# danspeech/danspeech

Hardware: AMD Instinct MI355X
Metric: audio-seconds/sec (RTFx) recognize() on 10 s clips, batch=32 (higher is better)
Workload: dtype f32 (two-term fp16 split operands, 3 MFMA products, fp32 accumulate)

## Files before the change

### danspeech_amd/csrc/api.hip

```cpp
#include "common.h"
#include "model.h"

#include <algorithm>
#include <cmath>
#include <cstring>
#include <cstdlib>
#include <mutex>
#include <fcntl.h>
#include <sys/file.h>
#include <unistd.h>

using namespace dsmi;

static thread_local std::string g_create_error;

#define HIP_OK(m, expr)                                                                   \
    do {                                                                                  \
        hipError_t e_ = (expr);                                                           \
        if (e_ != hipSuccess) {                                                           \
            (m)->err = std::string(#expr) + ": " + hipGetErrorString(e_);                 \
            return DSMI_ERR_HIP;                                                          \
        }                                                                                 \
    } while (0)

// ... 601 lines not shown
        return RingEnv{k && std::string(k) == "ring4", t ? std::atoi(t) : 4, c ? std::atoi(c) : 0};
    }();
    return env;
}

static RnnPlanInput rnn_plan_input(const dsmi_model* m, int B, bool split16) {
    RnnPlanInput in;
    in.geom = m->geom; in.geom16 = m->geom16; in.have16 = m->have16; in.split16 = split16;
    in.B = B; in.n_cus = m->n_cus; in.inflight = m->inflight; in.ring_windows = m->ring_windows; in.lane = m->lane;
    in.rnn_mode = m->rnn_mode; in.persist_gen = m->persist_gen; in.rnn_kernel = m->rnn_kernel; in.ring8 = m->ring8; in.ring4 = m->ring4;
    in.ring4_small_shapes = ring_env().small_shapes; in.ring4_most = ring_env().most; in.ring_slot_cap = ring_env().slot_cap;
    return in;
}

static bool run_rnn_plan(dsmi_model* m, const RnnPlan& plan, int l, int B, int To, int dst, double sumlen, hipStream_t s) {
    const double H = m->desc.rnn_hidden_size, GH = (double)m->geom.G * m->desc.rnn_hidden_size, Dd = m->geom.D;
    if (plan.launches[0].kernel == RNN_STEPS) {
        RnnStepLaunch st = rnn_step_launch(m, l, B, To, dst);
        for (int step = 0; step < To; ++step) {
            st.step = step;
            int act = 0;
            for (int i = 0; i < B; ++i) act += step < m->host_out_lens[i] ? 1 : 0;
            st.ev = timer_arm(m, KK_STEP, (step & 7) == 3, 2.0 * Dd * GH * H * act, 4.0 * Dd * (GH * H + (double)B * (GH + 2.0 * H)));
            launch_rnn_step(st, s);
        }
        m->last_plan_x16 = false; m->last_plan_n = 1; m->last_plan[0] = plan.launches[0];
        return true;
    }
    RnnPersist16Launch p16;
    RnnPersistLaunch p8;
    if (plan.x16) p16 = persist16_launch(m, l, B, To, dst);
    else p8 = persist_launch(m, l, B, To, dst);
    const size_t cnt_words = (size_t)m->geom.D * ceil_div(B, 16) * To * kPersist16CntWords;
    if (plan.x16) (void)hipMemsetAsync(m->pcnt, 0, sizeof(unsigned) * (cnt_words + 2 * ceil_div(B, 16) + 2), s);
    else (void)hipMemsetAsync(m->pcnt, 0, sizeof(unsigned) * (size_t)m->geom.D * ceil_div(B, 32) * To, s);
    static const bool ring_xcd = [] { const char* e = exp_env("DSMI_DEBUG_RING_XCD"); return !(e && e[0] == '0'); }();
    PersistGate* gate = persist_gate(m->device);
    std::unique_lock<std::mutex> turn(gate->mu, std::defer_lock);
    bool ok = true;
    for (int i = 0; i < plan.launches.size() && ok; ++i) {
        const RnnLaunch& L = plan.launches[i];
        const EvPair ev = timer_arm(m, KK_PERSIST, true, L.part * 2.0 * Dd * GH * H * sumlen, L.part * 4.0 * Dd * (GH * H + (double)To * B * (GH + 2.0 * H)));
        if (!L.join) {
            turn.lock();
            if (L.gate == GATE_RING) ring_gate_wait(gate, s, L.slot0, L.nslots, L.cus, m->n_cus);
            else gate_wait(gate, s, L.slot0, L.nslots);
        }
        p16.ev = ev;
        switch (L.kernel) {
            case RNN_PERSIST8: p8.ev = ev; p8.d0 = L.at; p8.ny = L.n; ok = launch_rnn_persist(p8, s); break;
            case RNN_PERSIST16: p16.pgroups = L.n; p16.waves = 8; ok = launch_rnn_persist16(p16, s); break;
            case RNN_PERSIST16_HALF: p16.pgroups = L.n; p16.waves = 4; ok = launch_rnn_persist16(p16, s); break;
            case RNN_DUO: p16.pair0 = L.at; p16.npairs = L.n; ok = launch_rnn_persist_duo(p16, s); break;
            default:
                p16.tile0 = L.at; p16.ntw = L.n; p16.nwin = L.nwin;
                p16.tickets = ring_xcd ? m->pcnt + cnt_words + L.ticket : nullptr;
                ok = L.kernel == RNN_RING8 ? launch_rnn_persist_ring(p16, s) : launch_rnn_persist_ring4(p16, s);
        }
        if (!ok || i + 1 == plan.launches.size() || !plan.launches[i + 1].join) {
            if (L.gate == GATE_RING) ring_gate_record(gate, s, L.slot0, L.nslots, L.cus);
            else gate_record(gate, s, L.slot0, L.nslots);
            turn.unlock();
        }
    }
    if (ok) {
        m->last_plan_x16 = plan.x16; m->last_plan_n = plan.launches.size();
        for (int i = 0; i < std::min(m->last_plan_n, (int)dsmi_model::kLastPlanKept); ++i) m->last_plan[i] = plan.launches[i];
    }
    return ok;
}

static void run_rnn_layer(dsmi_model* m, int l, GemmLaunch gl, int B, int To, int dst, hipStream_t s) {
    double sumlen = 0;
    for (int i = 0; i < B; ++i) sumlen += m->host_out_lens[i];
    const double GH = (double)m->geom.G * m->desc.rnn_hidden_size, Dd = m->geom.D;
    RnnPlanInput in = rnn_plan_input(m, B, m->gemm_mode == 1 && gl.w_sp);
    RnnPlan plan = plan_rnn_layer(in);
    if (plan.x16) {
        gl.w_sp = m->rnn[l].wih16_sp; gl.bias = m->rnn[l].bih16; gl.N = m->geom16.Np; gl.ldc = m->geom16.Np;
    }
    gl.ev = timer_arm(m, gl.mode == GEMM_A_CONV ? KK_GEMM0 : KK_GEMM, true, 2.0 * Dd * GH * gl.K * sumlen,
                      4.0 * ((double)gl.M * gl.K * (gl.a2 ? 2 : 1) + (double)gl.N * gl.K + (double)gl.M * gl.N));
    unsigned* sem = (dense_tokens() > 0 && m->inflight >= 2) ? dense_sem(m->device) : nullptr;
    if (sem) hipLaunchKernelGGL(dense_enter_kernel, dim3(1), dim3(64), 0, s, sem, (unsigned)dense_tokens());
    launch_gemm(gl, s);
    if (sem) hipLaunchKernelGGL(dense_leave_kernel, dim3(1), dim3(64), 0, s, sem);
    if (run_rnn_plan(m, plan, l, B, To, dst, sumlen, s)) return;
    if (plan.x16) {
        gl.w_sp = m->rnn[l].wih_sp; gl.bias = m->rnn[l].bih; gl.N = m->geom.Np; gl.ldc = m->geom.Np; gl.ev = EvPair{};
        launch_gemm(gl, s);
        in.have16 = false;
        plan = plan_rnn_layer(in);
        if (run_rnn_plan(m, plan, l, B, To, dst, sumlen, s)) return;
    }
    in.rnn_mode = 0;
    (void)run_rnn_plan(m, plan_rnn_layer(in), l, B, To, dst, sumlen, s);
}

static GemmLaunch xproj_gemm(dsmi_model* m, int l, int B, int To) {
    GemmLaunch gl{};
    const RnnW& r = m->rnn[l];
    gl.w = r.wih; gl.bias = r.bih; gl.c = m->xp;
    gl.w_sp = m->gemm_mode == 1 ? r.wih_sp : nullptr;
    gl.a_sp = m->a_sp;
    gl.M = To * B; gl.N = m->geom.Np; gl.K = r.K; gl.ldw = r.ldw; gl.ldc = m->geom.Np;
    gl.B = B; gl.T = To;
    return gl;
}

static int stage_lens(dsmi_model* m, int B, hipStream_t s) {
    if (B > m->stage_cap) {
        HIP_OK(m, hipDeviceSynchronize());
        if (m->lens_stage) (void)hipHostFree(m->lens_stage);
        m->lens_stage = nullptr;
        const int cap = std::max(B, 64);
        HIP_OK(m, hipHostMalloc((void**)&m->lens_stage, sizeof(int32_t) * (size_t)cap * dsmi_model::kStage, hipHostMallocDefault));
        m->stage_cap = cap;
        for (int i = 0; i < dsmi_model::kStage; ++i) {
            if (!m->stage_ev[i]) HIP_OK(m, hipEventCreateWithFlags(&m->stage_ev[i], hipEventDisableTiming));
            m->stage_used[i] = false;
        }
    }
    const int slot = m->stage_next++ % dsmi_model::kStage;
    if (m->stage_used[slot]) HIP_OK(m, hipEventSynchronize(m->stage_ev[slot]));
    int32_t* h = m->lens_stage + (size_t)slot * m->stage_cap;
    std::memcpy(h, m->host_out_lens.data(), sizeof(int32_t) * B);
    HIP_OK(m, hipMemcpyAsync(m->lens_dev, h, sizeof(int32_t) * B, hipMemcpyHostToDevice, s));
    HIP_OK(m, hipEventRecord(m->stage_ev[slot], s));
    m->stage_used[slot] = true;
    return DSMI_OK;
}

static int forward_enqueue(dsmi_model* m, const float* feat, int B, int T, float* probs, hipStream_t s);

static int persist_give_up(dsmi_model* m, hipStream_t s) {
    m->rnn_mode = 0;
    HIP_OK(m, hipMemsetAsync(m->perr, 0, sizeof(unsigned), s));
    return DSMI_OK;
}

static int collect_oldest(dsmi_model* m, bool recompute) {
    dsmi_model::FwdSlot& f = m->fwd[m->fwd_head];
    HIP_OK(m, hipEventSynchronize(f.done));
    m->fwd_head = (m->fwd_head + 1) % dsmi_model::kFwdRing;
    m->fwd_count -= 1;
    if (*f.err_host == 0) return DSMI_OK;
    *f.err_host = 0;
    hipStream_t s = (hipStream_t)f.stream;
    int rc;
    if ((rc = persist_give_up(m, s))) return rc;
    if (!recompute)
        return fail(m, DSMI_ERR_TIMEOUT, "the persistent recurrent kernel timed out in an earlier forward whose status was never "
                                         "collected with dsmi_forward_status: those results were invalid; this handle now runs "
                                         "one launch per step");
    m->host_out_lens.resize(f.B);
    for (int i = 0; i < f.B; ++i) m->host_out_lens[i] = seq_len(m, f.lens[i]);
    if ((rc = forward_enqueue(m, f.feat, f.B, f.T, f.probs, s))) return rc;
    HIP_OK(m, hipStreamSynchronize(s));
    m->recomputed += 1;
    m->err = "a hand-off wait of the persistent recurrent kernel timed out; the batch was recomputed with one launch per step";
    return DSMI_RECOMPUTED;
}

extern "C" int dsmi_forward(dsmi_model* m, const float* feat, const int32_t* lens, int B, int T, float* probs,
                            int32_t* out_lens, void* stream) {
    if (!m) return DSMI_ERR_INVALID;
    int rc = check_batch(m, lens, B, T);
// ... 371 lines not shown
```

### danspeech_amd/csrc/common.h

```cpp
#pragma once
#include <hip/hip_runtime.h>
#include <hip/hip_ext.h>
#include <cstdint>
#include <cstdio>
#include <cstdlib>
#include <string>
#include <vector>
#include <map>

#include "../../include/dsmi.h"
#include "rnn_plan.h"

namespace dsmi {

using f32x4 = __attribute__((ext_vector_type(4))) float;
using f32x16 = __attribute__((ext_vector_type(16))) float;

constexpr int kWave = 64;

struct EvPair { hipEvent_t start = nullptr, stop = nullptr; };
#define DSMI_LAUNCH(kern, grid, block, lds, stream, ev, ...)                                          \
    do {                                                                                              \
        if ((ev).start) hipExtLaunchKernelGGL(kern, grid, block, lds, stream, (ev).start, (ev).stop, 0, __VA_ARGS__); \
        else hipLaunchKernelGGL(kern, grid, block, lds, stream, __VA_ARGS__);                          \
    } while (0)

inline const char* exp_env(const char* name) {
#ifdef DSMI_EXPERIMENTS
    return std::getenv(name);
#else
    (void)name;
    return nullptr;
#endif
}

struct ConvSpec { int ci, co, kf, kt, sf, st, pf, pt; };
static const ConvSpec kConvSpecs[3] = {
    {1, 32, 41, 11, 2, 2, 20, 5},
    {32, 32, 21, 11, 2, 1, 10, 5},
    {32, 96, 21, 11, 2, 1, 10, 5},
};


struct ConvLaunch {
    const float* x; float* y; const float* wp; const float* bias; const float* bn_a; const float* bn_b;
    const int32_t* out_lens_dev;
    int B, ci, co, fi, fo, ti, to, xs, ys, layer;
    uint16_t* y_sp = nullptr;
    EvPair ev;
};
void launch_conv(const ConvLaunch& p, hipStream_t s);

struct ConvSplitLaunch {
    const uint16_t* x_sp;
    const uint16_t* wp_sp;
    const float* bias; const float* bn_a; const float* bn_b; const int32_t* out_lens_dev;
    float* y;
    uint16_t* y_sp;
    int B, co, fi, fo, ti, to, ys;
    EvPair ev;
};
void launch_conv_split(const ConvSplitLaunch& p, hipStream_t s);
std::vector<uint16_t> pack_conv_w_split(const float* w, int co_total);
std::vector<float> pack_conv_weights(const float* w, int layer);

std::vector<uint16_t> pack_conv1_w_split(const float* w);
void launch_conv1_split(const ConvLaunch& p, const uint16_t* wp_sp, hipStream_t s);

enum GemmAMode {
    GEMM_A_ROWMAJOR = 0,
    GEMM_A_SUM_BN = 1,
    GEMM_A_CONV = 2
};
struct GemmLaunch {
    int mode;
    const float* a; const float* a2; const float* alpha; const float* beta;
    const float* w; const float* bias; float* c;
    const uint16_t* w_sp = nullptr;
    uint16_t* a_sp = nullptr;
    int M, N, K;
    int lda, ldw, ldc;
    int B, T, ys;
    EvPair ev;
};
void launch_gemm(const GemmLaunch& p, hipStream_t s);
std::vector<uint16_t> pack_gemm_w_split(const float* w, int N, int K, int ldw);

int rnn_src_row(const RnnGeom& g, int packed_col, int* dir_out);
std::vector<float> pack_whh(const RnnGeom& g, const float* w_hh);
struct RnnStepLaunch {
    RnnGeom g;
    const float* whh_packed[2];
    const float* bhh[2];
    const float* xp;
    float* out[2];
    float* cstate[2];
    const int32_t* lens_dev;
    float* hpack;
    int B, T, step;
    const float* hcarry = nullptr;
    int pbase = 0;
    EvPair ev;
    unsigned long long* dbg = nullptr;
};
void launch_rnn_step(const RnnStepLaunch& p, hipStream_t s);

constexpr unsigned kPersistSpinLimit = 1u << 22;

struct RnnPersistLaunch {
    RnnGeom g;
    const uint16_t* whh_sp[2];
    const float* bhh[2]; const float* xp; float* out[2];
    const int32_t* lens_dev; uint16_t* hpack_sp;
    unsigned* counters;
    unsigned* err;
    int B, T;
    int d0 = 0, ny = 1;
    unsigned spin_limit = kPersistSpinLimit;
    int drop_wg = -1, drop_step = -1;
    EvPair ev;
    unsigned long long* dbg = nullptr;
    const float* h0 = nullptr;
    float* cst = nullptr;
};
std::vector<uint16_t> pack_whh_split(const RnnGeom& g, const float* w_hh);
bool launch_rnn_persist(const RnnPersistLaunch& p, hipStream_t s);

struct RnnPersist16Launch {
    RnnGeom g;
    const uint16_t* whh16[2];
    const float* bhh[2]; const float* xp; float* out[2];
    const int32_t* lens_dev; uint16_t* hpack16;
    unsigned* counters;
    unsigned* err;
    int B, T, pgroups;
    int waves = 8;
    int pair0 = 0, npairs = 0;
    int tile0 = 0, ntw = 0, nwin = 1;
    unsigned* tickets = nullptr;
    unsigned spin_limit = kPersistSpinLimit;
    int drop_wg = -1, drop_step = -1;
    EvPair ev;
    unsigned long long* dbg = nullptr;
};
constexpr int kPersist16Shards = 4;
constexpr int kPersist16CntWords = kPersist16Shards * 64;
std::vector<uint16_t> pack_whh16(const RnnGeom& g16, const float* w_hh);
size_t rnn_persist16_state_halfs(const RnnGeom& g16, int B);
bool launch_rnn_persist16(const RnnPersist16Launch& p, hipStream_t s);

bool launch_rnn_persist_duo(const RnnPersist16Launch& p, hipStream_t s);

bool launch_rnn_persist_ring(const RnnPersist16Launch& p, hipStream_t s);
bool launch_rnn_persist_ring4(const RnnPersist16Launch& p, hipStream_t s);

void launch_lookahead(const float* x, const float* w, float* y, int T, int B, int H, int context, hipStream_t s);
struct HeadLaunch {
    const float* x1; const float* x2; const float* bn_a; const float* bn_b;
    const float* w_packed; int H, C, T, B; float* probs;
    EvPair ev;
};
std::vector<float> pack_fc(const float* w, int C, int H);
void launch_head(const HeadLaunch& p, hipStream_t s);
void launch_greedy(const float* probs, const int32_t* sizes_dev, int B, int T, int C, int blank,
                   int32_t* raw, int32_t* ids, int32_t* offsets, int32_t* n_out, hipStream_t s);
void launch_add2(const float* a, const float* b, float* y, size_t rows, int H, int Hs, hipStream_t s);
void launch_pad_rows(const float* x, float* y, size_t rows, int I, int Is, hipStream_t s);
// ... 3 lines not shown
```

### danspeech_amd/csrc/conv1_split.hip

```cpp
#include "common.h"

namespace dsmi {

namespace {

using f16x8 = __attribute__((ext_vector_type(8))) _Float16;
using f16x4 = __attribute__((ext_vector_type(4))) _Float16;
using f16x2 = __attribute__((ext_vector_type(2))) _Float16;
using u32x4 = __attribute__((ext_vector_type(4))) unsigned int;
constexpr float kLoScale = 2048.f, kLoInv = 1.f / 2048.f;

constexpr int KF = 41, KT = 11, SF = 2, ST = 2, PF = 20, PT = 5, CO = 32;
constexpr int C1NF = 8;
constexpr int C1NT = C1NF * 64;
constexpr int C1TT = 64;
constexpr int ROWS = SF * (C1NF - 1) + KF;
constexpr int WIN = ST * (C1TT - 1) + KT + 5;
constexpr int PITCH = 144;
constexpr int COPY = ROWS * PITCH;
constexpr size_t C1_LDS = (size_t)2 * 2 * COPY * 2;

struct Conv1Args {
    const float* x; const uint16_t* wp; const float* bias; const float* bn_a; const float* bn_b; const int32_t* out_lens;
    float* y; uint16_t* y_sp;
    int B, fi, fo, ti, to, xs, ys;
};

template <bool SPLIT_OUT>
__global__ __launch_bounds__(C1NT, 4) void conv1_f16x3_kernel(Conv1Args p) {
    extern __shared__ __attribute__((aligned(16))) unsigned char c1sm[];
    _Float16* Xs = reinterpret_cast<_Float16*>(c1sm);
    const int tid = threadIdx.x, lane = tid & 63;
    const int wv = __builtin_amdgcn_readfirstlane(tid >> 6);
    const int li = lane & 31, hk = lane >> 5;
    const int t0 = blockIdx.x * C1TT, f0 = blockIdx.y * C1NF, b = blockIdx.z;
    const int f = f0 + wv;
    const int olen = p.out_lens[b];

    if (t0 >= olen) {
        if (SPLIT_OUT) {
            for (int idx = tid; idx < C1NF * 2 * C1TT * 4; idx += C1NT) {
                const int part = idx & 3, tl = (idx >> 2) % C1TT, pl = (idx / (4 * C1TT)) % 2, ff = idx / (4 * C1TT * 2);
                if (f0 + ff < p.fo && t0 + tl < p.to)
                    *reinterpret_cast<u32x4*>(reinterpret_cast<_Float16*>(p.y_sp) + ((((size_t)b * p.fo + f0 + ff) * 2 + pl) * p.to + t0 + tl) * 32 + part * 8) = u32x4{0, 0, 0, 0};
            }
        } else {
            for (int idx = tid; idx < CO * C1NF * C1TT; idx += C1NT) {
                const int tl = idx % C1TT, ff = (idx / C1TT) % C1NF, co = idx / (C1TT * C1NF);
                if (f0 + ff < p.fo && t0 + tl < p.to) p.y[(((size_t)b * CO + co) * p.fo + f0 + ff) * p.ys + t0 + tl] = 0.f;
            }
        }
        return;
    }

    const int fin0 = SF * f0 - PF, tin0 = ST * t0 - PT;
    for (int idx = tid; idx < ROWS * (PITCH / 2); idx += C1NT) {
        const int row = idx / (PITCH / 2), q = 2 * (idx - row * (PITCH / 2));
        const int fin = fin0 + row;
        float v[2] = {0.f, 0.f};
        if (fin >= 0 && fin < p.fi) {
            const float* src = p.x + ((size_t)b * p.fi + fin) * p.xs;
#pragma unroll
            for (int e = 0; e < 2; ++e) {
                const int tin = tin0 + q + e;
                if (tin >= 0 && tin < p.ti && q + e < WIN) v[e] = src[tin];
            }
        }
        f16x2 h, l;
#pragma unroll
        for (int e = 0; e < 2; ++e) {
            const _Float16 hi = (_Float16)v[e];
            h[e] = hi; l[e] = (_Float16)((v[e] - (float)hi) * kLoScale);
        }
        _Float16* r0 = Xs + row * PITCH + q;
        *reinterpret_cast<f16x2*>(r0) = h;
        *reinterpret_cast<f16x2*>(r0 + 2 * COPY) = l;
        if (q >= 2) {
            *reinterpret_cast<f16x2*>(r0 + COPY - 2) = h;
            *reinterpret_cast<f16x2*>(r0 + 3 * COPY - 2) = l;
        }
    }
    __syncthreads();
    if (f >= p.fo) return;

    f32x16 acc[2], acl[2];
#pragma unroll
    for (int tt = 0; tt < 2; ++tt)
#pragma unroll
        for (int r = 0; r < 16; ++r) { acc[tt][r] = 0.f; acl[tt][r] = 0.f; }

    const _Float16* xb = Xs + (SF * wv) * PITCH + 4 * li + 8 * hk;
    const u32x4* wq = reinterpret_cast<const u32x4*>(p.wp) + lane;
    u32x4 wn[2] = {wq[0], wq[64]};
#pragma unroll 1
    for (int kf = 0; kf < KF; ++kf) {
        const f16x8 wh = __builtin_bit_cast(f16x8, wn[0]), wl = __builtin_bit_cast(f16x8, wn[1]);
        if (kf + 1 < KF) { wn[0] = wq[(size_t)(kf + 1) * 128]; wn[1] = wq[(size_t)(kf + 1) * 128 + 64]; }
        const _Float16* xr = xb + kf * PITCH;
        f16x8 xh[2], xl[2];
#pragma unroll
        for (int tt = 0; tt < 2; ++tt) {
            const f16x4 a0 = *reinterpret_cast<const f16x4*>(xr + tt * COPY), a1 = *reinterpret_cast<const f16x4*>(xr + tt * COPY + 4);
            const f16x4 b0 = *reinterpret_cast<const f16x4*>(xr + (2 + tt) * COPY), b1 = *reinterpret_cast<const f16x4*>(xr + (2 + tt) * COPY + 4);
            xh[tt] = f16x8{a0[0], a0[1], a0[2], a0[3], a1[0], a1[1], a1[2], a1[3]};
            xl[tt] = f16x8{b0[0], b0[1], b0[2], b0[3], b1[0], b1[1], b1[2], b1[3]};
        }
#pragma unroll
        for (int tt = 0; tt < 2; ++tt) acl[tt] = __builtin_amdgcn_mfma_f32_32x32x16_f16(wl, xh[tt], acl[tt], 0, 0, 0);
#pragma unroll
        for (int tt = 0; tt < 2; ++tt) acc[tt] = __builtin_amdgcn_mfma_f32_32x32x16_f16(wh, xh[tt], acc[tt], 0, 0, 0);
#pragma unroll
        for (int tt = 0; tt < 2; ++tt) acl[tt] = __builtin_amdgcn_mfma_f32_32x32x16_f16(wh, xl[tt], acl[tt], 0, 0, 0);
    }

#pragma unroll
    for (int tt = 0; tt < 2; ++tt) {
        const int t = t0 + 2 * li + tt;
        if (t >= p.to) continue;
        if (SPLIT_OUT) {
#pragma unroll
            for (int g = 0; g < 4; ++g) {
                f16x4 h, l;
#pragma unroll
                for (int q = 0; q < 4; ++q) {
                    const int co = q + 8 * g + 4 * hk;
                    float v = (acc[tt][4 * g + q] + acl[tt][4 * g + q] * kLoInv + p.bias[co]) * p.bn_a[co] + p.bn_b[co];
                    v = fminf(fmaxf(v, 0.f), 20.f);
                    v = t < olen ? v : 0.f;
                    const _Float16 a = (_Float16)v;
                    h[q] = a; l[q] = (_Float16)(v - (float)a);
                }
                _Float16* base = reinterpret_cast<_Float16*>(p.y_sp) + ((((size_t)b * p.fo + f) * 2) * (size_t)p.to + t) * 32 + 8 * g + 4 * hk;
                *reinterpret_cast<f16x4*>(base) = h;
                *reinterpret_cast<f16x4*>(base + (size_t)p.to * 32) = l;
            }
        } else {
#pragma unroll
            for (int r = 0; r < 16; ++r) {
                const int co = (r & 3) + 8 * (r >> 2) + 4 * hk;
                float v = (acc[tt][r] + acl[tt][r] * kLoInv + p.bias[co]) * p.bn_a[co] + p.bn_b[co];
                v = fminf(fmaxf(v, 0.f), 20.f);
                p.y[(((size_t)b * CO + co) * p.fo + f) * p.ys + t] = t < olen ? v : 0.f;
            }
        }
    }
}

inline uint16_t c1_bits(_Float16 h) {
    uint16_t u;
    __builtin_memcpy(&u, &h, 2);
    return u;
}

}

std::vector<uint16_t> pack_conv1_w_split(const float* w) {
    std::vector<uint16_t> out((size_t)KF * 2 * 64 * 8, 0);
    for (int kf = 0; kf < KF; ++kf)
        for (int lane = 0; lane < 64; ++lane)
            for (int e = 0; e < 8; ++e) {
                const int co = lane & 31, kt = 8 * (lane >> 5) + e;
                if (kt >= KT) continue;
                const float x = w[((size_t)co * KF + kf) * KT + kt];
                const _Float16 h1 = (_Float16)x;
                const _Float16 h2 = (_Float16)((x - (float)h1) * kLoScale);
                const size_t base = (((size_t)kf * 2) * 64 + lane) * 8 + e;
                out[base] = c1_bits(h1); out[base + 512] = c1_bits(h2);
            }
    return out;
}

void launch_conv1_split(const ConvLaunch& c, const uint16_t* wp_sp, hipStream_t s) {
    Conv1Args a{c.x, wp_sp, c.bias, c.bn_a, c.bn_b, c.out_lens_dev, c.y, c.y_sp, c.B, c.fi, c.fo, c.ti, c.to, c.xs, c.ys};
    const dim3 grid(ceil_div(c.to, C1TT), ceil_div(c.fo, C1NF), c.B);
    if (c.y_sp) {
        (void)hipFuncSetAttribute(reinterpret_cast<const void*>(conv1_f16x3_kernel<true>), hipFuncAttributeMaxDynamicSharedMemorySize, (int)C1_LDS);
        DSMI_LAUNCH(conv1_f16x3_kernel<true>, grid, dim3(C1NT), C1_LDS, s, c.ev, a);
    } else {
        (void)hipFuncSetAttribute(reinterpret_cast<const void*>(conv1_f16x3_kernel<false>), hipFuncAttributeMaxDynamicSharedMemorySize, (int)C1_LDS);
        DSMI_LAUNCH(conv1_f16x3_kernel<false>, grid, dim3(C1NT), C1_LDS, s, c.ev, a);
// ... 5 lines not shown
```

### danspeech_amd/csrc/conv_split.hip

```cpp
#include "common.h"
#include <type_traits>

namespace dsmi {

namespace {

using f16x8 = __attribute__((ext_vector_type(8))) _Float16;
using f16x4 = __attribute__((ext_vector_type(4))) _Float16;
constexpr float kConvWScale = 64.f;
using u32x4 = __attribute__((ext_vector_type(4))) unsigned int;

constexpr int BNF = 4;
constexpr int BTT = 64;
constexpr int KT = 11, KF = 21, SF = 2, PF = 10, PT = 5, CI = 32;
constexpr int WIN = BTT + KT - 1;
constexpr int NPL = 2;
constexpr int PITCH = 32;
constexpr int ROWPLANE = WIN * PITCH;
constexpr int RCHUNK = NPL * WIN * 4;
constexpr int CPR = (RCHUNK + 255) / 256;
constexpr int NSLOT = 2 * BNF;

struct ConvSplitArgs {
    const uint16_t* x_sp; const uint16_t* wp_sp; const float* bias; const float* bn_a; const float* bn_b;
    const int32_t* out_lens; float* y; uint16_t* y_sp;
    int B, fi, fo, ti, to, ys;
    int nco;
};

__device__ __forceinline__ void store_split4(uint16_t* y_sp, size_t bf_index, int t_stride, int t, int c0, const float (&v)[4]) {
    f16x4 h, l;
#pragma unroll
    for (int c = 0; c < 4; ++c) {
        const _Float16 hi = (_Float16)v[c];
        h[c] = hi; l[c] = (_Float16)(v[c] - (float)hi);
    }
    _Float16* base = reinterpret_cast<_Float16*>(y_sp) + ((bf_index * NPL) * (size_t)t_stride + t) * 32 + c0;
    *reinterpret_cast<f16x4*>(base) = h;
    *reinterpret_cast<f16x4*>(base + (size_t)t_stride * 32) = l;
}

template <bool SPLIT_OUT, bool XPIPE = true>
__global__ __launch_bounds__(256, 2) void conv_f16x3_kernel(ConvSplitArgs p) {
    extern __shared__ __attribute__((aligned(16))) unsigned char csm[];
    _Float16* Xs = reinterpret_cast<_Float16*>(csm);
    const int tid = threadIdx.x, lane = tid & 63;
    const int wv = __builtin_amdgcn_readfirstlane(tid >> 6);
    const int t0 = blockIdx.x * BTT, f0 = blockIdx.y * BNF;
    const int b = blockIdx.z / p.nco, ct = blockIdx.z - b * p.nco;
    const int f = f0 + wv;
    const int olen = p.out_lens[b];
    const int CO = 32 * p.nco;

    if (t0 >= olen) {
        if (SPLIT_OUT) {
            for (int idx = tid; idx < BNF * NPL * BTT * 4; idx += 256) {
                const int part = idx & 3, tl = (idx >> 2) % BTT, pl = (idx / (4 * BTT)) % NPL, ff = idx / (4 * BTT * NPL);
                if (f0 + ff < p.fo && t0 + tl < p.to)
                    *reinterpret_cast<u32x4*>(reinterpret_cast<_Float16*>(p.y_sp) + ((((size_t)b * p.fo + f0 + ff) * NPL + pl) * p.to + t0 + tl) * 32 + part * 8) = u32x4{0, 0, 0, 0};
            }
        } else {
            for (int idx = tid; idx < 32 * BNF * BTT; idx += 256) {
                const int tl = idx % BTT, ff = (idx / BTT) % BNF, co = ct * 32 + idx / (BTT * BNF);
                if (f0 + ff < p.fo && t0 + tl < p.to) p.y[(((size_t)b * CO + co) * p.fo + f0 + ff) * p.ys + t0 + tl] = 0.f;
            }
        }
        return;
    }

    f32x4 acc[2][4];
#pragma unroll
    for (int c = 0; c < 2; ++c)
#pragma unroll
        for (int tt = 0; tt < 4; ++tt) acc[c][tt] = f32x4{0.f, 0.f, 0.f, 0.f};

    const int r0 = SF * f0 - PF;
    auto load_row = [&](int fin, u32x4 (&dst)[CPR]) {
#pragma unroll
        for (int i = 0; i < CPR; ++i) {
            const int c = tid + 256 * i;
            u32x4 v = {0, 0, 0, 0};
            if (c < RCHUNK) {
                const int part = c & 3, st = (c >> 2) % WIN, pl = (c >> 2) / WIN;
                const int tin = t0 - PT + st;
                if (fin >= 0 && fin < p.fi && tin >= 0 && tin < p.ti)
                    v = *reinterpret_cast<const u32x4*>(reinterpret_cast<const _Float16*>(p.x_sp) +
                                                        ((((size_t)b * p.fi + fin) * NPL + pl) * p.ti + tin) * 32 + part * 8);
            }
            dst[i] = v;
        }
    };
    auto store_row = [&](int slot8, const u32x4 (&src)[CPR]) {
#pragma unroll
        for (int i = 0; i < CPR; ++i) {
            const int c = tid + 256 * i;
            if (c < RCHUNK) {
                const int part = c & 3, st = (c >> 2) % WIN, pl = (c >> 2) / WIN;
                *reinterpret_cast<u32x4*>(Xs + (slot8 * NPL + pl) * ROWPLANE + st * PITCH + ((part ^ ((st >> 1) & 3)) * 8)) = src[i];
            }
        }
    };

    const u32x4* wbase = reinterpret_cast<const u32x4*>(p.wp_sp) + lane;
    const int l15 = lane & 15, l4 = lane >> 4;
    f16x8 wq[2][2][NPL];
    auto load_w = [&](int q, f16x8 (&dst)[2][NPL]) {
#pragma unroll
        for (int c = 0; c < 2; ++c)
#pragma unroll
            for (int pl = 0; pl < NPL; ++pl)
                dst[c][pl] = __builtin_bit_cast(f16x8, wbase[((((size_t)q * p.nco + ct) * 2 + c) * NPL + pl) * 64]);
    };
    constexpr int NQ = KF * KT;
    load_w(0, wq[0]);
    load_w(1, wq[1]);
    auto tap = [&](const _Float16* xrow, int kf, int kt, auto slot_c) {
        constexpr int slot = decltype(slot_c)::value;
        const int q = kf * KT + kt;
        f16x8 wf[2][NPL];
#pragma unroll
        for (int c = 0; c < 2; ++c)
#pragma unroll
            for (int pl = 0; pl < NPL; ++pl) wf[c][pl] = wq[slot][c][pl];
        load_w(min(q + 2, NQ - 1), wq[slot]);
        f16x8 xf[4][NPL];
#pragma unroll
        for (int tt = 0; tt < 4; ++tt) {
            const int st = tt * 16 + kt + l15;
#pragma unroll
            for (int pl = 0; pl < NPL; ++pl)
                xf[tt][pl] = *reinterpret_cast<const f16x8*>(xrow + pl * ROWPLANE + st * PITCH + ((l4 ^ ((st >> 1) & 3)) * 8));
        }
#pragma unroll
        for (int pp = 0; pp < 3; ++pp)
#pragma unroll
            for (int c = 0; c < 2; ++c)
#pragma unroll
                for (int tt = 0; tt < 4; ++tt)
                    acc[c][tt] = __builtin_amdgcn_mfma_f32_16x16x32_f16(wf[c][pp == 0 ? 1 : 0], xf[tt][pp == 1 ? 1 : 0], acc[c][tt], 0, 0, 0);
    };
    auto read_x = [&](const _Float16* xrow, int kt, f16x8 (&xf)[4][NPL]) {
        const int st0 = kt + l15;
        const _Float16* base = xrow + st0 * PITCH + ((l4 ^ ((st0 >> 1) & 3)) * 8);
#pragma unroll
        for (int pl = 0; pl < NPL; ++pl)
#pragma unroll
            for (int tt = 0; tt < 4; ++tt) xf[tt][pl] = *reinterpret_cast<const f16x8*>(base + pl * ROWPLANE + tt * 16 * PITCH);
    };
    auto tap_p = [&](const _Float16* xrow, int kf, int kt, auto slot_c, const f16x8 (&xf)[4][NPL], f16x8 (&xn)[4][NPL], bool more) {
        constexpr int slot = decltype(slot_c)::value;
        const int q = kf * KT + kt;
        f16x8 wf[2][NPL];
#pragma unroll
        for (int c = 0; c < 2; ++c)
#pragma unroll
            for (int pl = 0; pl < NPL; ++pl) wf[c][pl] = wq[slot][c][pl];
        load_w(min(q + 2, NQ - 1), wq[slot]);
        if (more) read_x(xrow, kt + 1, xn);
#pragma unroll
        for (int pp = 0; pp < 3; ++pp)
#pragma unroll
            for (int c = 0; c < 2; ++c)
#pragma unroll
                for (int tt = 0; tt < 4; ++tt)
                    acc[c][tt] = __builtin_amdgcn_mfma_f32_16x16x32_f16(wf[c][pp == 0 ? 1 : 0], xf[tt][pp == 1 ? 1 : 0], acc[c][tt], 0, 0, 0);
        if (more) {
#pragma unroll
            for (int g = 0; g < 8; ++g) {
                __builtin_amdgcn_sched_group_barrier(0x100, 1, 0);
                __builtin_amdgcn_sched_group_barrier(0x008, 3, 0);
            }
        }
    };
    auto taps = [&](const _Float16* xrow, int kf, auto first_slot) {
        constexpr int S0 = decltype(first_slot)::value;
        if constexpr (XPIPE) {
            f16x8 xa[4][NPL], xb[4][NPL];
            read_x(xrow, 0, xa);
#pragma unroll 1
            for (int kt = 0; kt + 1 < KT; kt += 2) {
                tap_p(xrow, kf, kt, std::integral_constant<int, S0>{}, xa, xb, true);
                tap_p(xrow, kf, kt + 1, std::integral_constant<int, S0 ^ 1>{}, xb, xa, true);
            }
            tap_p(xrow, kf, KT - 1, std::integral_constant<int, S0>{}, xa, xb, false);
        } else {
#pragma unroll 1
            for (int kt = 0; kt + 1 < KT; kt += 2) {
                tap(xrow, kf, kt, std::integral_constant<int, S0>{});
                tap(xrow, kf, kt + 1, std::integral_constant<int, S0 ^ 1>{});
            }
            tap(xrow, kf, KT - 1, std::integral_constant<int, S0>{});
        }
    };

    u32x4 stg[CPR];
    auto kernel_row = [&](int kf, auto first_slot) {
        const int fam = kf & 1, m0 = kf >> 1;
        if (kf >= 1 && kf + 1 < KF) store_row(((kf - 1) & 1) * 4 + (((kf - 1) >> 1) & 3), stg);
        if (kf + 2 < KF) load_row(r0 + kf + 8, stg);
        if (f < p.fo) taps(Xs + ((fam * 4 + ((m0 + wv) & 3)) * NPL) * ROWPLANE, kf, first_slot);
        __syncthreads();
    };
    {
        u32x4 pre[4][CPR];
#pragma unroll
        for (int half = 0; half < 2; ++half) {
#pragma unroll
            for (int j = 0; j < 4; ++j) load_row(r0 + half * 4 + j, pre[j]);
#pragma unroll
            for (int j = 0; j < 4; ++j) {
                const int row = half * 4 + j;
                store_row((row & 1) * 4 + (row >> 1), pre[j]);
            }
        }
    }
    __syncthreads();
    static_assert(KF % 2 == 1, "the last kernel row is an even one");
#pragma unroll 1
    for (int kf = 0; kf + 1 < KF; kf += 2) {
        kernel_row(kf, std::integral_constant<int, 0>{});
        kernel_row(kf + 1, std::integral_constant<int, 1>{});
    }
    kernel_row(KF - 1, std::integral_constant<int, 0>{});

    if (f >= p.fo) return;
#pragma unroll
    for (int tt = 0; tt < 4; ++tt) {
        const int t = t0 + tt * 16 + l15;
        if (t >= p.to) continue;
#pragma unroll
        for (int c = 0; c < 2; ++c) {
            float v[4];
#pragma unroll
            for (int q = 0; q < 4; ++q) {
                const int co = ct * 32 + c * 16 + 4 * l4 + q;
                float x = (acc[c][tt][q] * (1.f / kConvWScale) + p.bias[co]) * p.bn_a[co] + p.bn_b[co];
                x = fminf(fmaxf(x, 0.f), 20.f);
                v[q] = t < olen ? x : 0.f;
            }
            if (SPLIT_OUT) {
                store_split4(p.y_sp, (size_t)b * p.fo + f, p.to, t, c * 16 + 4 * l4, v);
            } else {
#pragma unroll
                for (int q = 0; q < 4; ++q)
                    p.y[(((size_t)b * CO + ct * 32 + c * 16 + 4 * l4 + q) * p.fo + f) * p.ys + t] = v[q];
            }
        }
    }
}

inline uint16_t c_f16_bits(_Float16 h) {
    uint16_t u;
    __builtin_memcpy(&u, &h, 2);
    return u;
}

}

std::vector<uint16_t> pack_conv_w_split(const float* w, int co_total) {
    const int nco = co_total / 32;
    std::vector<uint16_t> out((size_t)KF * KT * nco * 2 * NPL * 64 * 8, 0);
    for (int kf = 0; kf < KF; ++kf)
        for (int kt = 0; kt < KT; ++kt)
            for (int ct = 0; ct < nco; ++ct)
                for (int c = 0; c < 2; ++c)
                    for (int lane = 0; lane < 64; ++lane)
                        for (int e = 0; e < 8; ++e) {
                            const int co = ct * 32 + c * 16 + (lane & 15), ci = 8 * (lane >> 4) + e;
                            const float x = w[(((size_t)co * CI + ci) * KF + kf) * KT + kt] * kConvWScale;
                            const _Float16 h1 = (_Float16)x;
                            const _Float16 h2 = (_Float16)(x - (float)h1);
                            const size_t base = ((((((size_t)kf * KT + kt) * nco + ct) * 2 + c) * NPL) * 64 + lane) * 8 + e;
                            out[base] = c_f16_bits(h1); out[base + 512] = c_f16_bits(h2);
                        }
    return out;
}

void launch_conv_split(const ConvSplitLaunch& c, hipStream_t s) {
    ConvSplitArgs a{c.x_sp, c.wp_sp, c.bias, c.bn_a, c.bn_b, c.out_lens_dev, c.y, c.y_sp, c.B, c.fi, c.fo, c.ti, c.to, c.ys, c.co / 32};
    const dim3 grid(ceil_div(c.to, BTT), ceil_div(c.fo, BNF), c.B * a.nco);
    const size_t lds = (size_t)NSLOT * NPL * ROWPLANE * 2;
    (void)hipFuncSetAttribute(reinterpret_cast<const void*>(conv_f16x3_kernel<true>), hipFuncAttributeMaxDynamicSharedMemorySize, (int)lds);
    (void)hipFuncSetAttribute(reinterpret_cast<const void*>(conv_f16x3_kernel<false>), hipFuncAttributeMaxDynamicSharedMemorySize, (int)lds);
#ifdef DSMI_EXPERIMENTS
    static const bool plain = [] { const char* e = exp_env("DSMI_DEBUG_CONV_XPIPE"); return e && std::atoi(e) == 0; }();
    if (plain) {
        (void)hipFuncSetAttribute(reinterpret_cast<const void*>(conv_f16x3_kernel<true, false>), hipFuncAttributeMaxDynamicSharedMemorySize, (int)lds);
        (void)hipFuncSetAttribute(reinterpret_cast<const void*>(conv_f16x3_kernel<false, false>), hipFuncAttributeMaxDynamicSharedMemorySize, (int)lds);
        if (c.y_sp) DSMI_LAUNCH((conv_f16x3_kernel<true, false>), grid, dim3(256), lds, s, c.ev, a);
        else DSMI_LAUNCH((conv_f16x3_kernel<false, false>), grid, dim3(256), lds, s, c.ev, a);
        return;
    }
#endif
    if (c.y_sp) DSMI_LAUNCH((conv_f16x3_kernel<true>), grid, dim3(256), lds, s, c.ev, a);
    else DSMI_LAUNCH((conv_f16x3_kernel<false>), grid, dim3(256), lds, s, c.ev, a);
}

}
```

### danspeech_amd/csrc/gemm.hip

```cpp
#include "common.h"
#include <cstdlib>

namespace dsmi {

constexpr int BM = 128, BN = 128, BK = 32;
constexpr int LDT = BK + 4;
constexpr int LDC = BM + 4;

struct GemmArgs {
    const float* a; const float* a2; const float* alpha; const float* beta;
    const float* w; const float* bias; float* c;
    int M, N, K, lda, ldw, ldc, B, T, ys, tiles_per_b;
};

template <int MODE>
__global__ __launch_bounds__(256, 2) void gemm_f32_kernel(GemmArgs p) {
    extern __shared__ __attribute__((aligned(16))) float smem[];
    constexpr int A_TILE = (MODE == GEMM_A_CONV) ? BK * LDC : BM * LDT;
    constexpr int W_TILE = BN * LDT;
    constexpr int STAGE = A_TILE + W_TILE;

    const int tid = threadIdx.x;
    const int lane = tid & 63, wid = tid >> 6;
    const int wr = wid >> 1, wc = wid & 1;
// ... 375 lines not shown
            const int pp = e >> 5, mi = (e >> 3) & 3, ni = e & 7;
            if (e < 12 * GAP && e % GAP == 0) dma_piece(ktn, e / GAP);
            acc[mi][ni] = __builtin_amdgcn_mfma_f32_16x16x32_f16(af[mi][pp == 2 ? 1 : 0], wf[ni][pp == 1 ? 1 : 0], acc[mi][ni], 0, 0, 0);
        }
#pragma unroll
        for (int g = 0; g < 12; ++g) {
            __builtin_amdgcn_sched_group_barrier(0x010, 1, 0);
            __builtin_amdgcn_sched_group_barrier(0x008, GAP, 0);
        }
        __builtin_amdgcn_sched_group_barrier(0x008, 96 - 12 * GAP, 0);
        asm volatile("s_waitcnt vmcnt(0)\n\ts_barrier" ::: "memory");
    }

    int m0 = mt * BM, bb = 0, t0 = 0;
    if (CONV_ROWS) { bb = mt / p.tiles_per_b; t0 = (mt % p.tiles_per_b) * BM; }
    constexpr int TP = 68;
    float* turn = reinterpret_cast<float*>(lds) + wid * (16 * TP);
    const int cn = (lane & 15) * 4, cr = lane >> 4;
#pragma unroll
    for (int h = 0; h < 2; ++h) {
        if (2 * nt2 + h >= p.ntiles) break;
        const int n0 = (2 * nt2 + h) * BN;
        const int ncol = n0 + wc * 64 + cn;
        f32x4 bv = {0.f, 0.f, 0.f, 0.f};
        if (p.bias && ncol + 3 < p.N) bv = *reinterpret_cast<const f32x4*>(p.bias + ncol);
        else if (p.bias)
#pragma unroll
            for (int q = 0; q < 4; ++q) bv[q] = ncol + q < p.N ? p.bias[ncol + q] : 0.f;
#pragma unroll
        for (int mi = 0; mi < 4; ++mi) {
#pragma unroll
            for (int ni = 0; ni < 4; ++ni)
#pragma unroll
                for (int r = 0; r < 4; ++r) turn[((lane >> 4) * 4 + r) * TP + ni * 16 + (lane & 15)] = acc[mi][4 * h + ni][r];
            asm volatile("s_waitcnt lgkmcnt(0)" ::: "memory");
#pragma unroll
            for (int j = 0; j < 4; ++j) {
                const int i = wr * 64 + mi * 16 + cr + 4 * j;
                f32x4 v = *reinterpret_cast<const f32x4*>(turn + (cr + 4 * j) * TP + cn);
                v = v * (1.f / kGemmWScale) + bv;
                size_t crow;
                bool ok;
                if (CONV_ROWS) { ok = t0 + i < p.T; crow = (size_t)(t0 + i) * p.B + bb; }
                else { ok = m0 + i < p.M; crow = (size_t)(m0 + i); }
                if (!ok) continue;
                float* dst = p.c + crow * p.ldc + ncol;
                if (ncol + 3 < p.N) *reinterpret_cast<f32x4*>(dst) = v;
                else
#pragma unroll
                    for (int q = 0; q < 4; ++q)
                        if (ncol + q < p.N) dst[q] = v[q];
            }
            asm volatile("s_waitcnt lgkmcnt(0)" ::: "memory");
        }
    }
}

static inline uint16_t g_f16_bits(_Float16 h) {
    uint16_t u;
    __builtin_memcpy(&u, &h, 2);
    return u;
}

std::vector<uint16_t> pack_gemm_w_split(const float* w, int N, int K, int ldw) {
    const int ntl = ceil_div(N, BN), ktl = ceil_div(K, BK);
    std::vector<uint16_t> out((size_t)ntl * ktl * 2 * 128 * 32, 0);
    for (int n = 0; n < N; ++n)
        for (int k = 0; k < K; ++k) {
            const float x = w[(size_t)n * ldw + k] * kGemmWScale;
            const _Float16 h1 = (_Float16)x;
            const _Float16 h2 = (_Float16)(x - (float)h1);
            const size_t base = (((size_t)(n / BN) * ktl + k / BK) * 2) * 4096 + (size_t)(n % BN) * 32 + (k % BK);
            out[base] = g_f16_bits(h1); out[base + 4096] = g_f16_bits(h2);
        }
    return out;
}

static int gemm_panel_width(int ktiles) {
    static const int forced = [] { const char* e = exp_env("DSMI_DEBUG_GEMM_PN"); return e ? std::atoi(e) : 0; }();
    (void)ktiles;
    return forced > 0 ? forced : 5;
}

void launch_gemm(const GemmLaunch& g, hipStream_t s) {
    if (g.w_sp && g.a_sp) {
        GemmSplitArgs a;
        a.a = g.a; a.a2 = g.a2; a.alpha = g.alpha; a.beta = g.beta; a.w_sp = g.w_sp; a.bias = g.bias; a.c = g.c;
        a.M = g.M; a.N = g.N; a.K = g.K; a.lda = g.lda; a.ldc = g.ldc; a.B = g.B; a.T = g.T; a.ys = g.ys;
        a.tiles_per_b = 0; a.ktiles = ceil_div(g.K, BK);
        int mtiles3;
        if (g.mode == GEMM_A_CONV) { a.tiles_per_b = ceil_div(g.T, BM); mtiles3 = a.tiles_per_b * g.B; }
        else mtiles3 = ceil_div(g.M, BM);
        const dim3 sgrid(a.ktiles, mtiles3);
        switch (g.mode) {
            case GEMM_A_ROWMAJOR: hipLaunchKernelGGL(split_a_kernel<GEMM_A_ROWMAJOR>, sgrid, dim3(256), 0, s, a, g.a_sp); break;
            case GEMM_A_SUM_BN: hipLaunchKernelGGL(split_a_kernel<GEMM_A_SUM_BN>, sgrid, dim3(256), 0, s, a, g.a_sp); break;
            default: hipLaunchKernelGGL(split_a_kernel<GEMM_A_CONV>, sgrid, dim3(256), 0, s, a, g.a_sp); break;
        }
        a.ntiles = ceil_div(g.N, BN); a.mtiles = mtiles3;
        a.pn = gemm_panel_width(a.ktiles);
        const dim3 grid3(8 * ceil_div(a.ntiles * a.mtiles, 8));
        static const int wide = [] { const char* e = exp_env("DSMI_DEBUG_GEMM_WIDE"); return e ? std::atoi(e) : 1; }();
        static const bool pn_forced = exp_env("DSMI_DEBUG_GEMM_PN") != nullptr;
        a.pn2 = pn_forced ? std::max(1, (a.pn + 1) / 2) : 3;
#ifndef DSMI_EXPERIMENTS
        (void)wide; (void)grid3;
        {
#else
        if (wide) {
#endif
            const int ntiles2 = (a.ntiles + 1) / 2;
            const dim3 gridw(8 * ceil_div(ntiles2 * a.mtiles, 8));
            const size_t ldsw = 49152;
            if (g.mode == GEMM_A_CONV) DSMI_LAUNCH(gemm_f16x3_wide_kernel<true>, gridw, dim3(256), ldsw, s, g.ev, a, (const uint16_t*)g.a_sp);
            else DSMI_LAUNCH(gemm_f16x3_wide_kernel<false>, gridw, dim3(256), ldsw, s, g.ev, a, (const uint16_t*)g.a_sp);
            return;
        }
#ifdef DSMI_EXPERIMENTS
        static const int stages = [] { const char* e = exp_env("DSMI_DEBUG_GEMM_STAGES"); return e && std::atoi(e) == 2 ? 2 : 1; }();
        if (stages == 2) {
            const size_t lds2 = 65536;
            static bool attr = false;
            if (!attr) {
                (void)hipFuncSetAttribute(reinterpret_cast<const void*>(gemm_f16x3_kernel<true, 2>), hipFuncAttributeMaxDynamicSharedMemorySize, (int)lds2);
                (void)hipFuncSetAttribute(reinterpret_cast<const void*>(gemm_f16x3_kernel<false, 2>), hipFuncAttributeMaxDynamicSharedMemorySize, (int)lds2);
                attr = true;
            }
            if (g.mode == GEMM_A_CONV) DSMI_LAUNCH((gemm_f16x3_kernel<true, 2>), grid3, dim3(256), lds2, s, g.ev, a, (const uint16_t*)g.a_sp);
            else DSMI_LAUNCH((gemm_f16x3_kernel<false, 2>), grid3, dim3(256), lds2, s, g.ev, a, (const uint16_t*)g.a_sp);
            return;
        }
        const size_t lds3 = 32768;
        if (g.mode == GEMM_A_CONV) DSMI_LAUNCH((gemm_f16x3_kernel<true, 1>), grid3, dim3(256), lds3, s, g.ev, a, (const uint16_t*)g.a_sp);
        else DSMI_LAUNCH((gemm_f16x3_kernel<false, 1>), grid3, dim3(256), lds3, s, g.ev, a, (const uint16_t*)g.a_sp);
        return;
#endif
    }
    GemmArgs a;
    a.a = g.a; a.a2 = g.a2; a.alpha = g.alpha; a.beta = g.beta; a.w = g.w; a.bias = g.bias; a.c = g.c;
    a.M = g.M; a.N = g.N; a.K = g.K; a.lda = g.lda; a.ldw = g.ldw; a.ldc = g.ldc;
    a.B = g.B; a.T = g.T; a.ys = g.ys; a.tiles_per_b = 0;
    int mtiles;
    if (g.mode == GEMM_A_CONV) {
        a.tiles_per_b = ceil_div(g.T, BM);
        mtiles = a.tiles_per_b * g.B;
    } else {
        mtiles = ceil_div(g.M, BM);
    }
    dim3 grid(ceil_div(g.N, BN), mtiles);
    const size_t lds_rm = 2 * (BM * LDT + BN * LDT) * sizeof(float);
    const size_t lds_cv = 2 * (BK * LDC + BN * LDT) * sizeof(float);
    switch (g.mode) {
        case GEMM_A_ROWMAJOR:
            DSMI_LAUNCH(gemm_f32_kernel<GEMM_A_ROWMAJOR>, grid, dim3(256), lds_rm, s, g.ev, a); break;
        case GEMM_A_SUM_BN:
            DSMI_LAUNCH(gemm_f32_kernel<GEMM_A_SUM_BN>, grid, dim3(256), lds_rm, s, g.ev, a); break;
        default:
            DSMI_LAUNCH(gemm_f32_kernel<GEMM_A_CONV>, grid, dim3(256), lds_cv, s, g.ev, a); break;
    }
}

}
```

Measured before the change: 60200.

## Skip out-of-range conv kernel rows and move A-split outside dense semaphore

Result: no change. 60330, median of 2 (+0.2%).

```diff
diff --git a/danspeech_amd/csrc/api.hip b/danspeech_amd/csrc/api.hip
--- a/danspeech_amd/csrc/api.hip
+++ b/danspeech_amd/csrc/api.hip
@@ -707,7 +707,10 @@
     gl.ev = timer_arm(m, gl.mode == GEMM_A_CONV ? KK_GEMM0 : KK_GEMM, true, 2.0 * Dd * GH * gl.K * sumlen,
                       4.0 * ((double)gl.M * gl.K * (gl.a2 ? 2 : 1) + (double)gl.N * gl.K + (double)gl.M * gl.N));
     unsigned* sem = (dense_tokens() > 0 && m->inflight >= 2) ? dense_sem(m->device) : nullptr;
+    static const bool split_inside = [] { const char* e = exp_env("DSMI_DEBUG_SPLIT_IN_TOKEN"); return e && std::atoi(e) == 1; }();
+    if (!split_inside) launch_split_a(gl, s);
     if (sem) hipLaunchKernelGGL(dense_enter_kernel, dim3(1), dim3(64), 0, s, sem, (unsigned)dense_tokens());
+    if (split_inside) launch_split_a(gl, s);
     launch_gemm(gl, s);
     if (sem) hipLaunchKernelGGL(dense_leave_kernel, dim3(1), dim3(64), 0, s, sem);
     if (run_rnn_plan(m, plan, l, B, To, dst, sumlen, s)) return;
diff --git a/danspeech_amd/csrc/common.h b/danspeech_amd/csrc/common.h
--- a/danspeech_amd/csrc/common.h
+++ b/danspeech_amd/csrc/common.h
@@ -83,6 +83,7 @@
     int B, T, ys;
     EvPair ev;
 };
+void launch_split_a(const GemmLaunch& p, hipStream_t s);
 void launch_gemm(const GemmLaunch& p, hipStream_t s);
 std::vector<uint16_t> pack_gemm_w_split(const float* w, int N, int K, int ldw);
 
diff --git a/danspeech_amd/csrc/conv1_split.hip b/danspeech_amd/csrc/conv1_split.hip
--- a/danspeech_amd/csrc/conv1_split.hip
+++ b/danspeech_amd/csrc/conv1_split.hip
@@ -91,11 +91,12 @@
 
     const _Float16* xb = Xs + (SF * wv) * PITCH + 4 * li + 8 * hk;
     const u32x4* wq = reinterpret_cast<const u32x4*>(p.wp) + lane;
-    u32x4 wn[2] = {wq[0], wq[64]};
+    const int kf_lo = max(0, PF - SF * f), kf_hi = min(KF, p.fi + PF - SF * f);
+    u32x4 wn[2] = {wq[(size_t)kf_lo * 128], wq[(size_t)kf_lo * 128 + 64]};
 #pragma unroll 1
-    for (int kf = 0; kf < KF; ++kf) {
+    for (int kf = kf_lo; kf < kf_hi; ++kf) {
         const f16x8 wh = __builtin_bit_cast(f16x8, wn[0]), wl = __builtin_bit_cast(f16x8, wn[1]);
-        if (kf + 1 < KF) { wn[0] = wq[(size_t)(kf + 1) * 128]; wn[1] = wq[(size_t)(kf + 1) * 128 + 64]; }
+        if (kf + 1 < kf_hi) { wn[0] = wq[(size_t)(kf + 1) * 128]; wn[1] = wq[(size_t)(kf + 1) * 128 + 64]; }
         const _Float16* xr = xb + kf * PITCH;
         f16x8 xh[2], xl[2];
 #pragma unroll
diff --git a/danspeech_amd/csrc/conv_split.hip b/danspeech_amd/csrc/conv_split.hip
--- a/danspeech_amd/csrc/conv_split.hip
+++ b/danspeech_amd/csrc/conv_split.hip
@@ -40,7 +40,7 @@
     *reinterpret_cast<f16x4*>(base + (size_t)t_stride * 32) = l;
 }
 
-template <bool SPLIT_OUT, bool XPIPE = true>
+template <bool SPLIT_OUT, bool XPIPE = true, bool FULL_WALK = false>
 __global__ __launch_bounds__(256, 2) void conv_f16x3_kernel(ConvSplitArgs p) {
     extern __shared__ __attribute__((aligned(16))) unsigned char csm[];
     _Float16* Xs = reinterpret_cast<_Float16*>(csm);
@@ -75,6 +75,10 @@
         for (int tt = 0; tt < 4; ++tt) acc[c][tt] = f32x4{0.f, 0.f, 0.f, 0.f};
 
     const int r0 = SF * f0 - PF;
+    const int flast = min(f0 + BNF, p.fo) - 1;
+    const int kf_lo = FULL_WALK ? 0 : max(0, PF - SF * flast), kf_hi = FULL_WALK ? KF : min(KF, p.fi + PF - SF * f0);
+    const int wlo = FULL_WALK || f >= p.fo ? 0 : max(0, PF - SF * f);
+    const int whi = f >= p.fo ? 0 : (FULL_WALK ? KF : min(KF, p.fi + PF - SF * f));
     auto load_row = [&](int fin, u32x4 (&dst)[CPR]) {
 #pragma unroll
         for (int i = 0; i < CPR; ++i) {
@@ -112,8 +116,8 @@
                 dst[c][pl] = __builtin_bit_cast(f16x8, wbase[((((size_t)q * p.nco + ct) * 2 + c) * NPL + pl) * 64]);
     };
     constexpr int NQ = KF * KT;
-    load_w(0, wq[0]);
-    load_w(1, wq[1]);
+    load_w(wlo * KT + (wlo & 1), wq[0]);
+    load_w(wlo * KT + 1 - (wlo & 1), wq[1]);
     auto tap = [&](const _Float16* xrow, int kf, int kt, auto slot_c) {
         constexpr int slot = decltype(slot_c)::value;
         const int q = kf * KT + kt;
@@ -196,9 +200,9 @@
     u32x4 stg[CPR];
     auto kernel_row = [&](int kf, auto first_slot) {
         const int fam = kf & 1, m0 = kf >> 1;
-        if (kf >= 1 && kf + 1 < KF) store_row(((kf - 1) & 1) * 4 + (((kf - 1) >> 1) & 3), stg);
-        if (kf + 2 < KF) load_row(r0 + kf + 8, stg);
-        if (f < p.fo) taps(Xs + ((fam * 4 + ((m0 + wv) & 3)) * NPL) * ROWPLANE, kf, first_slot);
+        if (kf > kf_lo && kf + 1 < kf_hi) store_row(((kf - 1) & 1) * 4 + (((kf - 1) >> 1) & 3), stg);
+        if (kf + 2 < kf_hi) load_row(r0 + kf + 8, stg);
+        if (kf >= wlo && kf < whi) taps(Xs + ((fam * 4 + ((m0 + wv) & 3)) * NPL) * ROWPLANE, kf, first_slot);
         __syncthreads();
     };
     {
@@ -206,22 +210,23 @@
 #pragma unroll
         for (int half = 0; half < 2; ++half) {
 #pragma unroll
-            for (int j = 0; j < 4; ++j) load_row(r0 + half * 4 + j, pre[j]);
+            for (int j = 0; j < 4; ++j) load_row(r0 + kf_lo + half * 4 + j, pre[j]);
 #pragma unroll
             for (int j = 0; j < 4; ++j) {
-                const int row = half * 4 + j;
-                store_row((row & 1) * 4 + (row >> 1), pre[j]);
+                const int row = kf_lo + half * 4 + j;
+                store_row((row & 1) * 4 + ((row >> 1) & 3), pre[j]);
             }
         }
     }
     __syncthreads();
-    static_assert(KF % 2 == 1, "the last kernel row is an even one");
+    int kf = kf_lo;
+    if (kf & 1) { kernel_row(kf, std::integral_constant<int, 1>{}); ++kf; }
 #pragma unroll 1
-    for (int kf = 0; kf + 1 < KF; kf += 2) {
+    for (; kf + 1 < kf_hi; kf += 2) {
         kernel_row(kf, std::integral_constant<int, 0>{});
         kernel_row(kf + 1, std::integral_constant<int, 1>{});
     }
-    kernel_row(KF - 1, std::integral_constant<int, 0>{});
+    if (kf < kf_hi) kernel_row(kf, std::integral_constant<int, 0>{});
 
     if (f >= p.fo) return;
 #pragma unroll
@@ -283,6 +288,14 @@
     (void)hipFuncSetAttribute(reinterpret_cast<const void*>(conv_f16x3_kernel<true>), hipFuncAttributeMaxDynamicSharedMemorySize, (int)lds);
     (void)hipFuncSetAttribute(reinterpret_cast<const void*>(conv_f16x3_kernel<false>), hipFuncAttributeMaxDynamicSharedMemorySize, (int)lds);
 #ifdef DSMI_EXPERIMENTS
+    static const bool full = [] { const char* e = exp_env("DSMI_DEBUG_CONV_FULLWALK"); return e && std::atoi(e) == 1; }();
+    if (full) {
+        (void)hipFuncSetAttribute(reinterpret_cast<const void*>(conv_f16x3_kernel<true, true, true>), hipFuncAttributeMaxDynamicSharedMemorySize, (int)lds);
+        (void)hipFuncSetAttribute(reinterpret_cast<const void*>(conv_f16x3_kernel<false, true, true>), hipFuncAttributeMaxDynamicSharedMemorySize, (int)lds);
+        if (c.y_sp) DSMI_LAUNCH((conv_f16x3_kernel<true, true, true>), grid, dim3(256), lds, s, c.ev, a);
+        else DSMI_LAUNCH((conv_f16x3_kernel<false, true, true>), grid, dim3(256), lds, s, c.ev, a);
+        return;
+    }
     static const bool plain = [] { const char* e = exp_env("DSMI_DEBUG_CONV_XPIPE"); return e && std::atoi(e) == 0; }();
     if (plain) {
         (void)hipFuncSetAttribute(reinterpret_cast<const void*>(conv_f16x3_kernel<true, false>), hipFuncAttributeMaxDynamicSharedMemorySize, (int)lds);
diff --git a/danspeech_amd/csrc/gemm.hip b/danspeech_amd/csrc/gemm.hip
--- a/danspeech_amd/csrc/gemm.hip
+++ b/danspeech_amd/csrc/gemm.hip
@@ -481,22 +481,31 @@
     return forced > 0 ? forced : 5;
 }
 
+static GemmSplitArgs gemm_split_args(const GemmLaunch& g) {
+    GemmSplitArgs a{};
+    a.a = g.a; a.a2 = g.a2; a.alpha = g.alpha; a.beta = g.beta; a.w_sp = g.w_sp; a.bias = g.bias; a.c = g.c;
+    a.M = g.M; a.N = g.N; a.K = g.K; a.lda = g.lda; a.ldc = g.ldc; a.B = g.B; a.T = g.T; a.ys = g.ys;
+    a.tiles_per_b = 0; a.ktiles = ceil_div(g.K, BK);
+    if (g.mode == GEMM_A_CONV) { a.tiles_per_b = ceil_div(g.T, BM); a.mtiles = a.tiles_per_b * g.B; }
+    else a.mtiles = ceil_div(g.M, BM);
+    a.ntiles = ceil_div(g.N, BN);
+    return a;
+}
+
+void launch_split_a(const GemmLaunch& g, hipStream_t s) {
+    if (!(g.w_sp && g.a_sp)) return;
+    const GemmSplitArgs a = gemm_split_args(g);
+    const dim3 sgrid(a.ktiles, a.mtiles);
+    switch (g.mode) {
+        case GEMM_A_ROWMAJOR: hipLaunchKernelGGL(split_a_kernel<GEMM_A_ROWMAJOR>, sgrid, dim3(256), 0, s, a, g.a_sp); break;
+        case GEMM_A_SUM_BN: hipLaunchKernelGGL(split_a_kernel<GEMM_A_SUM_BN>, sgrid, dim3(256), 0, s, a, g.a_sp); break;
+        default: hipLaunchKernelGGL(split_a_kernel<GEMM_A_CONV>, sgrid, dim3(256), 0, s, a, g.a_sp); break;
+    }
+}
+
 void launch_gemm(const GemmLaunch& g, hipStream_t s) {
     if (g.w_sp && g.a_sp) {
-        GemmSplitArgs a;
-        a.a = g.a; a.a2 = g.a2; a.alpha = g.alpha; a.beta = g.beta; a.w_sp = g.w_sp; a.bias = g.bias; a.c = g.c;
-        a.M = g.M; a.N = g.N; a.K = g.K; a.lda = g.lda; a.ldc = g.ldc; a.B = g.B; a.T = g.T; a.ys = g.ys;
-        a.tiles_per_b = 0; a.ktiles = ceil_div(g.K, BK);
-        int mtiles3;
-        if (g.mode == GEMM_A_CONV) { a.tiles_per_b = ceil_div(g.T, BM); mtiles3 = a.tiles_per_b * g.B; }
-        else mtiles3 = ceil_div(g.M, BM);
-        const dim3 sgrid(a.ktiles, mtiles3);
-        switch (g.mode) {
-            case GEMM_A_ROWMAJOR: hipLaunchKernelGGL(split_a_kernel<GEMM_A_ROWMAJOR>, sgrid, dim3(256), 0, s, a, g.a_sp); break;
-            case GEMM_A_SUM_BN: hipLaunchKernelGGL(split_a_kernel<GEMM_A_SUM_BN>, sgrid, dim3(256), 0, s, a, g.a_sp); break;
-            default: hipLaunchKernelGGL(split_a_kernel<GEMM_A_CONV>, sgrid, dim3(256), 0, s, a, g.a_sp); break;
-        }
-        a.ntiles = ceil_div(g.N, BN); a.mtiles = mtiles3;
+        GemmSplitArgs a = gemm_split_args(g);
         a.pn = gemm_panel_width(a.ktiles);
         const dim3 grid3(8 * ceil_div(a.ntiles * a.mtiles, 8));
         static const int wide = [] { const char* e = exp_env("DSMI_DEBUG_GEMM_WIDE"); return e ? std::atoi(e) : 1; }();
```
